# HeadReaper-hc/PL-inertial-slam

Measured on AMD Instinct MI355X. Metric: local-BA iterations/sec (50 KF, 20k pts, 4k lines, IMU), higher is better.
Workload: dtype f64; 1 GPU; configs[2]: 50 KF / 20k points / 4k lines + IMU preintegration edges (9-DoF PVR + 6-DoF bias vertices); K=50, points=20000, lines=4000, point_obs=86023, line_obs=17197, pose_dim=735, dense_dim=357, banded_twisted_solve=False, twin_factorisation=True, fused_landmark_passes=True

## Files before the change

pl-inertial-slam_amd/csrc/plba_api.hip:

```cpp
#include <atomic>
#include <algorithm>
#include <thread>
#include <array>
#include <chrono>
#include <cmath>
#include <cstdio>
#include <cstring>
#include <condition_variable>
#include <functional>
#include <map>
#include <mutex>

#include "plba_problem.h"

using namespace plba;

namespace {
char g_create_err[256] = "";
static std::mutex g_ctx_mu;
static std::vector<HostCtx> g_ctx_free;
static std::map<int, hipStream_t> g_lib_stream;
static std::vector<plba_problem*> g_parked;
static const size_t PARK_MAX = 2;
}
// ... 464 lines not shown
        if (use_lut) for (int w = 0; w < g.nw; ++w) lut[g.kf[w]] = (uint8_t)w;
        int l = g.lm0, ob = H.span_ob0[gi];
        for (int n = H.span_at[gi]; n < H.span_end[gi]; ++n, ++l) {
            const int s = ordall[n];
            o_slot[l] = s; o_fixed[l] = fixed[s]; o_ob0[l] = ob;
            uint8_t* w8 = o_ws8 + (size_t)l * wmax;
            memset(w8, 0xFF, (size_t)wmax);
            int nk = 0;
            for (int e = ls[s]; e < ls[s + 1]; ++e, ++ob, ++nk) {
                int w = 0;
                if (use_lut) w = lut[okf[e]];
                else while (g.kf[w] != okf[e]) ++w;
                bad |= (w8[w] != 0xFF);
                w8[w] = (uint8_t)nk;
                o_orig[ob] = e;
            }
        }
    }
    if (bad) H.bad[t] = 1;
}
static bool lm_groups_finish(LmHost& H) {
    HostPool::get().finish();
    for (int b : H.bad) if (b) return false;
    return true;
}
static void build_lm_groups(const plba_problem* p, const std::vector<int32_t>& lm_start, const std::vector<int32_t>& ob_kf, LmHost& H) {
    const int K = p->win.K, Np = p->win.Np, Nl = p->win.Nl, Ep = p->win.Ep, L = Np + Nl, E = (int)ob_kf.size();
    H.cov.assign((size_t)K * K, 0);
    const bool gt = (p->opt.diag & PLBA_DIAG_TIMING) != 0;
    auto g0 = std::chrono::steady_clock::now();
    auto glap = [&](const char* what) { if (!gt) return; auto t = std::chrono::steady_clock::now(); fprintf(stderr, "[prepare]   groups: %-18s %8.3f ms\n", what, std::chrono::duration<double, std::milli>(t - g0).count()); g0 = t; };
    int nwide_pt = 0, nwide_ln = 0;
    for (int s = 0; s < L; ++s) if (lm_start[s + 1] - lm_start[s] > LMF_W) ++(s < Np ? nwide_pt : nwide_ln);
    const bool any_wide = nwide_pt + nwide_ln > 0;
    int steps = 1;
    {
        static int cus = 0;
        if (!cus) { int dev = 0; if (hipGetDevice(&dev) != hipSuccess || hipDeviceGetAttribute(&cus, hipDeviceAttributeMultiprocessorCount, dev) != hipSuccess || cus < 1) cus = 256; }
        const int slots = 2 * cus;
        const long wg_steps = (Np - nwide_pt + 31) / 32 + (Nl - nwide_ln + 15) / 16 + (nwide_pt + 15) / 16 + (nwide_ln + 7) / 8;
        const long cap1 = std::max<long>(32, (long)(1.12 * cus) - (p->win.M + 1) - (p->win.M / 4 + 1));
        steps = (int)std::max<long>(1, (wg_steps + cap1 - 1) / cap1);
        if (steps > 16) {
            for (int R = 1; R <= 64; ++R) {
                const long cap = (long)(0.97 * R * slots);
                steps = (int)std::max<long>(1, (wg_steps + cap - 1) / cap);
                if (steps <= 16) break;
// ... 106 lines not shown
    H.staged = false;
    if (nob > 20000) {
        H.p_ob_orig = (int32_t*)stage_take(std::max<size_t>(H.n_ob, 1) * 4);
        H.p_lm_slot = (int32_t*)stage_take(std::max<size_t>(H.n_lm, 1) * 4); H.p_lm_ob0 = (int32_t*)stage_take((H.n_lm + 1) * 4);
        H.p_lm_ws8 = (uint8_t*)stage_take(std::max<size_t>(H.n_lm * H.wmax, 1)); H.p_lm_fixed = (uint8_t*)stage_take(std::max<size_t>(H.n_lm, 1));
        H.staged = H.p_ob_orig && H.p_lm_slot && H.p_lm_ob0 && H.p_lm_ws8 && H.p_lm_fixed;
    }
    if (!H.staged) {
        H.lm_slot.resize(nlm); H.lm_ob0.resize(nlm + 1); H.lm_ws8.resize((size_t)nlm * H.wmax); H.lm_fixed.resize(nlm); H.ob_orig.resize(nob);
        H.p_lm_slot = H.lm_slot.data(); H.p_lm_ob0 = H.lm_ob0.data(); H.p_lm_ws8 = H.lm_ws8.data(); H.p_lm_fixed = H.lm_fixed.data(); H.p_ob_orig = H.ob_orig.data();
    }
    H.p_lm_ob0[nlm] = nob;
    const int NT = E > 400000 ? 32 : E > 60000 ? 16 : E > 20000 ? 4 : 1;
    H.gcut.assign(NT + 1, ngrp);
    H.gcut[0] = 0;
    for (int t = 1, g = 0; t < NT; ++t) { while (g < ngrp && H.span_ob0[g] < (int64_t)nob * t / NT) ++g; H.gcut[t] = g; }
    H.bad.assign(NT, 0);
    glap("table allocation");
    const plba_problem* pp = p; const std::vector<int32_t>* ls = &lm_start; const std::vector<int32_t>* ok = &ob_kf; LmHost* Hp = &H;
    HostPool::get().start(NT, [pp, ls, ok, Hp](int t) { lm_fill_groups(pp, *ls, *ok, *Hp, t); });
    {
        size_t npairs_tot = 0, nrows_tot = 0;
        for (const LmGroup& g : H.grp) { int nf = 0; for (int q = 0; q < g.nw; ++q) nf += g.off[q] >= 0; npairs_tot += (size_t)nf * (nf + 1) / 2; nrows_tot += nf; }
        H.blk_c.resize(npairs_tot); H.row_c.resize(nrows_tot);
        auto* bc = H.blk_c.data(); auto* rc = H.row_c.data();
        uint8_t* cov = H.cov.data();
        for (int gi = 0; gi < ngrp; ++gi) {
            const LmGroup& g = H.grp[gi];
            for (int q = 0; q < g.nw; ++q) {
                if (g.off[q] < 0) continue;
                for (int pp = 0; pp <= q; ++pp) {
                    if (g.off[pp] < 0) continue;
                    const int i = g.kf[pp], j = g.kf[q];
                    cov[(size_t)i * K + j] = 1; cov[(size_t)j * K + i] = 1;
                    *bc++ = {(int64_t)i * K + j, gi * H.npair + q * (q + 1) / 2 + pp};
                }
                *rc++ = {(int64_t)g.kf[q], gi * H.wmax + q};
            }
        }
    }
    {
        std::vector<int32_t>& c2 = H.c2; std::vector<int32_t>& pos = H.pos;
        c2.assign((size_t)K * K + 1, 0);
        for (const auto& b : H.blk_c) c2[b.first + 1]++;
        for (size_t k = 0; k < (size_t)K * K; ++k) c2[k + 1] += c2[k];
        H.blk_src.resize(H.blk_c.size());
        for (size_t k = 0; k < (size_t)K * K; ++k) if (c2[k + 1] > c2[k]) { const int i = (int)(k / K), j = (int)(k % K); H.blk_ij.push_back((int32_t)(i | (j << 16))); H.blk_start.push_back(c2[k]); }
        H.blk_start.push_back((int32_t)H.blk_c.size());
        pos.assign(c2.begin(), c2.end() - 1);
        for (const auto& b : H.blk_c) H.blk_src[pos[b.first]++] = b.second;
        c2.assign(K + 1, 0);
        for (const auto& r : H.row_c) c2[r.first + 1]++;
        for (int k = 0; k < K; ++k) c2[k + 1] += c2[k];
        H.row_src.resize(H.row_c.size());
        for (int k = 0; k < K; ++k) if (c2[k + 1] > c2[k]) { H.row_kf.push_back(k); H.row_start.push_back(c2[k]); }
        H.row_start.push_back((int32_t)H.row_c.size());
        pos.assign(c2.begin(), c2.end() - 1);
        for (const auto& r : H.row_c) H.row_src[pos[r.first]++] = r.second;
    }
    glap("gather lists");
// ... 1901 lines not shown
        const int o = w == "err_pvr" ? 0 : 9, nn = w == "err_pvr" ? 9 : 6;
        v.resize((size_t)p->win.M * nn);
        for (int m = 0; m < p->win.M; ++m) memcpy(&v[(size_t)m * nn], &h[(size_t)m * 16 + o], nn * 8);
    } else if (w == "err_prior") { HIPCK(p, fetch(d.pr_err, p->pr_nv ? p->pr_n : 0, v)); }
    else if ((w == "err_pt" || w == "err_ln") && p->lm_ok) {
        std::vector<double> h; HIPCK(p, fetch(p->d_ob_err.p, 2 * (size_t)p->E, h));
        if (w == "err_pt") v.assign(h.begin(), h.begin() + 2 * (size_t)p->win.Ep);
        else { v.assign((size_t)p->win.El * 3, 0.0); for (int e = 0; e < p->win.El; ++e) { v[3 * (size_t)e] = h[2 * (size_t)(p->win.Ep + e)]; v[3 * (size_t)e + 1] = h[2 * (size_t)(p->win.Ep + e) + 1]; } }
    }
    else if (w == "err_pt" || w == "err_ln") {
        std::vector<double> h; HIPCK(p, fetch(d.erec, ((size_t)p->win.Ep + 2 * (size_t)p->win.El) * EREC_UNIT, h));
        if (w == "err_pt") { v.resize((size_t)p->win.Ep * 2); for (int e = 0; e < p->win.Ep; ++e) { const size_t o = (size_t)p->ob_pos[e] * EREC_UNIT; v[2 * (size_t)e] = h[o + EREC_PT_E0]; v[2 * (size_t)e + 1] = h[o + EREC_PT_E0 + 1]; } }
        else { v.assign((size_t)p->win.El * 3, 0.0); for (int e = 0; e < p->win.El; ++e) { const size_t o = (size_t)p->ob_pos[p->win.Ep + e] * EREC_UNIT; v[3 * (size_t)e] = h[o + 13]; v[3 * (size_t)e + 1] = h[o + 14]; } }
    } else if (w == "erec") {
        if (p->lm_ok) FAIL(p, PLBA_ERR_STATE, "\"erec\": the fused landmark passes keep no record table");
        HIPCK(p, fetch(d.erec, ((size_t)p->win.Ep + 2 * (size_t)p->win.El) * EREC_UNIT, v));
    }
    else if (w == "stamps") { HIPCK(p, fetch(d.maxd_part, 80, v)); }
    else if (w == "dbgbuf") { HIPCK(p, fetch(d.dbgbuf, 128, v)); }
    else if (w == "pose_dim") v = {(double)p->P};
    else if (w == "marg_path") v.assign(p->marg_path, p->marg_path + 5);
    else if (w == "prof_lin_launches") v = {(double)p->prof_lin_launches};
    else if (w == "lm_groups") v = p->lm_hist;
    else if (w == "lm_fused") v = {(double)(p->lm_ok ? 1 : 0), (double)p->lv.ngrp, (double)p->lv.nblk, p->lm_ok && p->lm_hist.size() > 18 ? p->lm_hist[18] : 0.0 };
    else if (w == "marg_J") v = p->marg_dbg;
    else if (w == "dense_dim") v = {(double)(p->chain_ok ? p->cv.Pd : p->P)};
    else if (w == "band") v = {(double)(p->band_ok ? 1 : 0)};
    else if (w == "twin") v = {(double)(p->twin_ok ? 1 : 0)};
    else if (w == "solver_plan") {
        const bool ninv = !p->band_ok && (p->chain_ok ? p->dd.Ninv : p->dv.Ninv) != nullptr;
        v = {(double)(p->band_ok ? 3 : p->twin_ok ? 2 : p->chain_ok ? 1 : 0), (double)((p->chain_ok ? p->cv.Pdpad : p->Ppad) / 32), ninv ? 1.0 : 0.0, (double)p->plan_hbt,
             p->plan_twin[0], p->plan_twin[1], p->plan_twin[2], p->plan_twin[3], p->plan_twin[4], (double)(p->band_ok ? p->bandv.nA : 0), (double)(p->band_ok ? p->bandv.nB : 0)};
    }
    else if (w == "fact_launches_estimate") v = {(double)p->seg_launch_est};
    else if (w == "fact_launches") {
        if (p->band_ok) v = {2.0};
        else if (p->twin_ok) v = {(double)(p->twinv.nlaunch + (p->twinv.T - p->twinv.m0 - 1))};
        else v = {-1.0};
    }
    else if (w == "chi2") { HIPCK(p, plba_d2h(p, p->h_ctrl, d.ctrl, sizeof(Ctrl))); v = {p->h_ctrl->current_chi}; }
    else if (w == "maxdiag") { HIPCK(p, plba_d2h(p, p->h_ctrl, d.ctrl, sizeof(Ctrl))); v = {p->h_ctrl->maxdiag}; }
    else if (w == "solver_ok") { HIPCK(p, plba_d2h(p, p->h_ctrl, d.ctrl, sizeof(Ctrl))); v = {(double)p->h_ctrl->solver_ok}; }
    else FAIL(p, PLBA_ERR_INVALID, "debug_get: unknown buffer '%s'", what);
    if (n) *n = v.size();
    if (out) { const size_t c = std::min(v.size(), cap); if (c) memcpy(out, v.data(), c * 8); }
    return PLBA_OK;
// ... 4 lines not shown
```

pl-inertial-slam_amd/csrc/plba_internal.h:

```cpp
#pragma once
#include <hip/hip_runtime.h>
#include <stdint.h>
#include <map>
#include <mutex>
#include <string>
#include <utility>
#include <vector>

#include "plba.h"
#include "plba_math.h"

namespace plba {

constexpr int TILE = 64;

inline hipError_t ensure_dyn_lds(const void* func, int bytes) {
    static std::mutex mu;
    static std::map<std::pair<int, const void*>, int> done;
    int dev = 0;
    hipError_t e = hipGetDevice(&dev);
    if (e != hipSuccess) return e;
    std::lock_guard<std::mutex> lk(mu);
    auto it = done.find({dev, func});
    if (it != done.end() && it->second >= bytes) return hipSuccess;
// ... 69 lines not shown
    int band;
    int twin_m0;
    const int32_t* cs_order;
    const int32_t* twin_fac;
    const int32_t* perm;
    const int32_t* xmap;
    double* wtw;
    double* alt2;
    double* alt;
    int flow;
    int wide;
    double *chi_part, *scale_part, *maxd_part, *kfdiag, *posediag;
    Ctrl* ctrl;
    plba_trace_row* trace;
    int trace_cap;
    int* trace_n;
};

struct Robust { int on[5]; double delta[5]; };

constexpr int LMF_W = 8;
constexpr int LMF_W2 = 16;
struct LmGroup { int32_t lm0, nlm, nw, kind ; int32_t kf[LMF_W2]; int32_t off[LMF_W2]; };
struct LmView {
    int ngrp;
    const LmGroup* grp;
    const int32_t* lm_slot;
    const int32_t* lm_ob0;
    const int32_t* ob_orig;
    double* ob_chi_g;
    int wmax, npair, part_stride;
    const uint8_t* lm_ws8;
    const uint8_t* lm_fixed_g;
    uint8_t* ob_level_g;
    const double* meas_pt;
    const double* meas_ln;
    const double* ob_wt;
    double* part;
    int nblk;
    const int32_t* blk_ij;
    const int32_t* blk_start;
    const int32_t* blk_src;
    int nrow;
    const int32_t* row_kf;
    const int32_t* row_start;
    const int32_t* row_src;
// ... 106 lines not shown
```

pl-inertial-slam_amd/csrc/plba_kernels.hip:

```cpp
#include "plba_internal.h"
#include "plba_chain_dev.h"

namespace plba {

#define DEV __device__ __forceinline__

DEV double wave_sum(double v) {
#pragma unroll
    for (int o = 32; o > 0; o >>= 1) v += __shfl_down(v, o, 64);
    return v;
}
DEV double wave_max(double v) {
#pragma unroll
    for (int o = 32; o > 0; o >>= 1) v = fmax(v, __shfl_down(v, o, 64));
    return v;
}
DEV double block_sum_256(double v, double* s4) {
    v = wave_sum(v);
    int w = threadIdx.x >> 6;
    if ((threadIdx.x & 63) == 0) s4[w] = v;
    __syncthreads();
    double r = 0;
    if (threadIdx.x == 0) r = (s4[0] + s4[1]) + (s4[2] + s4[3]);
    __syncthreads();
// ... 1497 lines not shown
    hipLaunchKernelGGL(k_reduce, dim3(1), dim3(256), 0, s, d, nred, nred, owns_pose_edges ? 1 : 0, red);
}
void launch_posediag(const DevBuf& d, hipStream_t s) {
    hipLaunchKernelGGL(k_posediag, dim3((d.ld + 255) / 256), dim3(256), 0, s, d);
    hipLaunchKernelGGL(k_posediag_kf, dim3((d.K * 6 + 255) / 256), dim3(256), 0, s, d);
}
__global__ __launch_bounds__(256) void k_lm_lambda_init(DevBuf d, LmView lv, LmParams lp, double* red, int iteration, int nred) {
    __shared__ double s4[4];
    __shared__ double s_part[256];
    reduce_inline(d, nred, nred, red, s4);
    for (int r = threadIdx.x; r < d.ld; r += 256) d.posediag[r] = (r < d.P) ? d.Himu[(size_t)r * d.ld + r] + d.Hconst[(size_t)r * d.ld + r] : 0.0;
    __syncthreads();
    const int nent = lv.nrow * 6;
    const int nch = nent > 0 && nent <= 128 ? 256 / nent : 1;
    for (int base = 0; base < nent; base += 256) {
        const int idx = base + (int)threadIdx.x % (nch > 1 ? nent : 256), ch = nch > 1 ? (int)threadIdx.x / nent : 0;
        double v = 0.0;
        const bool live = idx < nent && ch < nch;
        int k = 0, c = 0;
        if (live) {
            k = idx / 6; c = idx - 6 * k;
            for (int q = lv.row_start[k] + ch; q < lv.row_start[k + 1]; q += nch) {
                const int src = lv.row_src[q];
                v += lv.part[(size_t)(src / lv.wmax) * lv.part_stride + lv.npair * 36 + (src % lv.wmax) * 12 + c];
            }
        }
        if (nch > 1) {
            s_part[threadIdx.x] = v;
            __syncthreads();
            if (live && ch == 0) { v = 0.0; for (int q = 0; q < nch; ++q) v += s_part[q * nent + idx]; }
        }
        if (live && ch == 0) {
            const int kf = lv.row_kf[k], o = d.kf_off_pvr[kf];
            d.kfdiag[kf * 6 + c] = v;
            if (o >= 0) d.posediag[o + pmap(c)] += v;
        }
    }
    __syncthreads();
    double md = 0.0;
    for (int r = threadIdx.x; r < d.P; r += 256) md = fmax(md, fabs(d.posediag[r]));
    double mx = block_max_256(md, s4);
    if (threadIdx.x == 0) {
        Ctrl* c = d.ctrl;
        c->current_chi = red[0];
        c->iteration = iteration;
        c->trial = 0;
        mx = fmax(mx, red[2]);
// ... 148 lines not shown
```

pl-inertial-slam_amd/csrc/plba_lm_dev.h:

```cpp
#pragma once

namespace plba {

typedef double double4v_lm __attribute__((ext_vector_type(4)));

constexpr int LMF_UNITS = 32;
constexpr int LMF_ROWS = 6 * LMF_W;
constexpr int LMF_SCOLS = 3 * LMF_UNITS;
constexpr int LMF_HCOLS = 2 * LMF_UNITS;
struct LmLds {
    double kc[2][LMF_W2][KFCAM_STRIDE];
    double xs[LMF_W2][6];
    double red[4][8];
    int koff[LMF_W2];
};
struct LmAcc {
    double op[4 * 24 * LMF_ROWS];
};

DEV double quad_or_sum(double v) { return quad_sum(v); }
DEV int quad_or_i(int v) {
    v |= __builtin_amdgcn_update_dpp(0, v, 0xB1, 0xf, 0xf, false);
    v |= __builtin_amdgcn_update_dpp(0, v, 0x4E, 0xf, 0xf, false);
    v |= __builtin_amdgcn_update_dpp(0, v, 0x141, 0xf, 0xf, false);
    return v;
}
DEV double shfl_xor8(double v) {
    return dpp_get<0x128, 0xf>(v);
}

DEV double lm_rcp(double x) {
    double y = __builtin_amdgcn_rcp(x);
    double e = fma(-x, y, 1.0);
    y = fma(y, e, y);
    e = fma(-x, y, 1.0);
    return fma(y, e, y);
}
DEV double lm_rsqrt(double x) {
    double y = __builtin_amdgcn_rsq(x);
    const double hx = 0.5 * x;
    y = y * fma(-hx * y, y, 1.5);
// ... 113 lines not shown
    if (s.has) {
        s.orig = lv.ob_err ? lv.ob_orig[s.e] : 0; s.wt = lv.ob_wt[s.e];
        s.lvl0 = lv.ob_level_g[s.e] == 0;
        if (IS_LINE) { const double* m = lv.meas_ln + (size_t)(s.e - d.Ep) * 3; s.meas[0] = m[0]; s.meas[1] = m[1]; s.meas[2] = m[2]; }
        else { const double2 m = reinterpret_cast<const double2*>(lv.meas_pt)[s.e]; s.meas[0] = m.x; s.meas[1] = m.y; }
    }
}
template <bool IS_LINE, bool WIDE = false>
DEV void lm_load(const DevBuf& d, const LmView& lv, const LmHead& g, int state, int step, int wv, int lane, LmStep& s) {
    LmIdx x;
    lm_load_idx<IS_LINE, WIDE>(lv, g, step, wv, lane, x);
    lm_load_data<IS_LINE, WIDE>(d, lv, state, lane, x, s);
}

DEV void lm_stage_window(const DevBuf& d, const LmGroup* gp, int nw, int state, LmLds& S) {
    if ((int)threadIdx.x < LMF_W2) {
        const int p = threadIdx.x;
        if (p < nw) { kfcam_make(d.cam, d.kf[state] + (size_t)gp->kf[p] * KF_STRIDE, S.kc[0][p]); S.koff[p] = gp->off[p]; }
        else { for (int t = 0; t < KFCAM_STRIDE; ++t) S.kc[0][p][t] = 0.0; S.koff[p] = -1; }
    }
}

constexpr int LMF_WCOLS = 24;
constexpr int LMF_NVEC = 33;
DEV void lm_wave_sync() {
    __builtin_amdgcn_fence(__ATOMIC_RELEASE, "wavefront");
    __builtin_amdgcn_wave_barrier();
    __builtin_amdgcn_fence(__ATOMIC_ACQUIRE, "wavefront");
}
template <bool IS_LINE, int MODE>
DEV void lm_schur_group(const DevBuf& d, const LmView& lv, const int gidx, const int state, const Robust& rb, LmLds& S, LmAcc& A4) {
    constexpr int NR = IS_LINE ? 1 : 2;
    const LmGroup* gp = lv.grp + gidx;
    const LmHead g = lm_head(*gp);
    const int wv = threadIdx.x >> 6, lane = threadIdx.x & 63, sub = lane & 7, li = lane & 15, lk = lane >> 4, u8 = lane >> 3;
    const double lambda = MODE == 0 ? d.ctrl->lambda : 0.0;
    lm_stage_window(d, gp, g.nw, state, S);
    const int nunits = IS_LINE ? 2 * g.nlm : g.nlm;
    const int nsteps = (nunits + LMF_UNITS - 1) / LMF_UNITS;
#ifdef PLBA_STAMPS_LMF
    unsigned long long fs[12] = {0,0,0,0,0,0,0,0,0,0,0,0}; fs[0] = __builtin_readcyclecounter();
#define FSTAMP(i) do { if (step == 0) fs[i] = __builtin_readcyclecounter(); } while (0)
#define FSTAMP1(i) fs[i] = __builtin_readcyclecounter()
#else
#define FSTAMP(i) do {} while (0)
#define FSTAMP1(i) do {} while (0)
#endif
    LmStep cur;
    lm_load<IS_LINE>(d, lv, g, state, 0, wv, lane, cur);
    LmIdx ix1;
    ix1.uvalid = false; ix1.slot = 0; ix1.e = 0; ix1.has = false; ix1.fixed = true;
    if (nsteps > 1) lm_load_idx<IS_LINE>(lv, g, 1, wv, lane, ix1);
    __syncthreads();
    const double* kc = S.kc[0][sub];
    const bool kfree = S.koff[sub] >= 0;
    const double4v_lm z4 = (double4v_lm){0.0, 0.0, 0.0, 0.0};
    double4v_lm a00 = z4, a10 = z4, a11 = z4, a20 = z4, a21 = z4, a22 = z4;
    double vec[LMF_NVEC];
#pragma unroll
    for (int t = 0; t < LMF_NVEC; ++t) vec[t] = 0.0;
    double chi_acc = 0.0, maxd = 0.0;
    double* op = A4.op + wv * (LMF_WCOLS * LMF_ROWS);
    for (int step = 0; step < nsteps; ++step) {
        FSTAMP(1);
        LmRows<NR> r;
        const int rowsel = IS_LINE ? (u8 & 1) : 0;
        lm_eval<IS_LINE, NR>(d, rb, kc, cur.has && kfree, cur.L, cur.meas, cur.wt, cur.has, cur.lvl0, rowsel, true, r);
        FSTAMP(2);
        double h[6], b[3];
        int nact;
        lm_hll<NR>(r, h, b, nact);
        FSTAMP(3);
        const bool active = cur.uvalid && nact > 0 && !cur.fixed;
        if (!IS_LINE || rowsel == 0) chi_acc += r.rho;
        if (MODE == 1 && r.act && (!IS_LINE || rowsel == 0)) {
            lv.ob_chi_g[cur.e] = r.chi;
            if (lv.ob_err) { lv.ob_err[2 * (size_t)cur.orig] = r.e[0]; }
        }
        if (MODE == 1 && lv.ob_err && r.act) lv.ob_err[2 * (size_t)cur.orig + (IS_LINE ? rowsel : 1)] = r.e[NR - 1];
        if (lv.dbg_out && cur.uvalid && sub == 0) {
            const int dslot = lv.lm_grouped ? lv.lm_slot[cur.slot] : cur.slot;
            double* ho = d.hll + (size_t)dslot * 12 + (IS_LINE ? 6 * rowsel : 0);
            double* bo = d.bl + (size_t)dslot * 6 + (IS_LINE ? 3 * rowsel : 0);
#pragma unroll
            for (int t = 0; t < 6; ++t) ho[t] = h[t];
// ... 44 lines not shown
                }
                double q = 0.0;
#pragma unroll
                for (int a = 0; a < NR; ++a) q += r.j[a][c] * es[a];
                vec[21 + c] -= q;
                vec[27 + c] += A3[0] * y[0] + A3[1] * y[1] + A3[2] * y[2];
#pragma unroll
                for (int c2 = 0; c2 <= c; ++c2) {
                    double hq = 0.0;
#pragma unroll
                    for (int a = 0; a < NR; ++a) hq += r.j[a][c] * r.j[a][c2];
#ifndef PLBA_X_NOH
                    vec[hidx++] += hq;
#else
                    (void)hq; (void)hidx;
#endif
                }
            }
            FSTAMP(4);
            LmStep nxt;
            if (step + 1 < nsteps) lm_load_data<IS_LINE>(d, lv, state, lane, ix1, nxt);
            if (step + 2 < nsteps) lm_load_idx<IS_LINE>(lv, g, step + 2, wv, lane, ix1);
            lm_wave_sync();
#pragma unroll 2
            for (int s4 = 0; s4 < LMF_WCOLS / 4; ++s4) {
                const double* col = op + (4 * s4 + lk) * LMF_ROWS + li;
                const double f0 = col[0], f1 = col[16], f2 = col[32];
#ifdef PLBA_X_NOMFMA
                a00[0] += f0 * f1 * f2;
                continue;
#endif
                a00 = __builtin_amdgcn_mfma_f64_16x16x4f64(f0, f0, a00, 0, 0, 0);
                a10 = __builtin_amdgcn_mfma_f64_16x16x4f64(f1, f0, a10, 0, 0, 0);
                a11 = __builtin_amdgcn_mfma_f64_16x16x4f64(f1, f1, a11, 0, 0, 0);
                a20 = __builtin_amdgcn_mfma_f64_16x16x4f64(f2, f0, a20, 0, 0, 0);
                a21 = __builtin_amdgcn_mfma_f64_16x16x4f64(f2, f1, a21, 0, 0, 0);
                a22 = __builtin_amdgcn_mfma_f64_16x16x4f64(f2, f2, a22, 0, 0, 0);
            }
            FSTAMP(5);
            lm_wave_sync();
            cur = nxt;
        }
        FSTAMP(7);
    }
    FSTAMP1(8);
#pragma unroll
    for (int t = 0; t < LMF_NVEC; ++t) {
        double v = vec[t];
        v += shfl_xor8(v);
        v += __shfl_xor(v, 16);
        v += __shfl_xor(v, 32);
        vec[t] = v;
    }
    chi_acc = wave_sum(chi_acc); maxd = wave_max(maxd);
    __syncthreads();
    double* cb = A4.op;
    double* vs = A4.op + 2 * 6 * 256;
    if (lane < LMF_W) {
#pragma unroll
        for (int t = 0; t < LMF_NVEC; ++t) vs[(wv * LMF_W + lane) * LMF_NVEC + t] = vec[t];
    }
    if (lane == 0) { S.red[wv][0] = chi_acc; S.red[wv][1] = maxd; }
    if (MODE == 0) {
        double* mine = cb + (wv & 1) * (6 * 256);
        if (wv < 2) {
#pragma unroll
            for (int v4 = 0; v4 < 4; ++v4) {
                const int o = (lk + 4 * v4) * 16 + li;
                mine[0 * 256 + o] = a00[v4]; mine[1 * 256 + o] = a10[v4]; mine[2 * 256 + o] = a11[v4];
                mine[3 * 256 + o] = a20[v4]; mine[4 * 256 + o] = a21[v4]; mine[5 * 256 + o] = a22[v4];
            }
        }
        __syncthreads();
        if (wv >= 2) {
#pragma unroll
            for (int v4 = 0; v4 < 4; ++v4) {
                const int o = (lk + 4 * v4) * 16 + li;
                mine[0 * 256 + o] += a00[v4]; mine[1 * 256 + o] += a10[v4]; mine[2 * 256 + o] += a11[v4];
                mine[3 * 256 + o] += a20[v4]; mine[4 * 256 + o] += a21[v4]; mine[5 * 256 + o] += a22[v4];
            }
        }
    }
    __syncthreads();
    FSTAMP1(9);
    double* part = lv.part + (size_t)gidx * lv.part_stride;
    if (MODE == 0) {
        for (int idx = threadIdx.x; idx < 36 * 36; idx += 256) {
            const int t = idx / 36, rc = idx - t * 36, r = rc / 6, c = rc - r * 6;
            const int q = (t >= 28) ? 7 : (t >= 21) ? 6 : (t >= 15) ? 5 : (t >= 10) ? 4 : (t >= 6) ? 3 : (t >= 3) ? 2 : (t >= 1) ? 1 : 0;
            const int p = t - q * (q + 1) / 2;
            int a = 6 * p + r, b2 = 6 * q + c;
            if (a < b2) { const int tmp = a; a = b2; b2 = tmp; }
            const int ta = a >> 4, tb = b2 >> 4;
            const int o = (ta * (ta + 1) / 2 + tb) * 256 + (a & 15) * 16 + (b2 & 15);
            const double sv = cb[o] + cb[6 * 256 + o];
            double hv = 0.0;
            if (p == q) {
                const int hr = r >= c ? r : c, hc = r >= c ? c : r, k = hr * (hr + 1) / 2 + hc;
                hv = (vs[(0 * LMF_W + p) * LMF_NVEC + k] + vs[(1 * LMF_W + p) * LMF_NVEC + k]) + (vs[(2 * LMF_W + p) * LMF_NVEC + k] + vs[(3 * LMF_W + p) * LMF_NVEC + k]);
            }
            part[idx] = hv - sv;
        }
    }
    if ((int)threadIdx.x < LMF_W * 12 && (MODE == 0 || threadIdx.x % 12 < 6)) {
        const int p = threadIdx.x / 12, k = 21 + threadIdx.x % 12;
        part[lv.npair * 36 + threadIdx.x] = (vs[(0 * LMF_W + p) * LMF_NVEC + k] + vs[(1 * LMF_W + p) * LMF_NVEC + k]) + (vs[(2 * LMF_W + p) * LMF_NVEC + k] + vs[(3 * LMF_W + p) * LMF_NVEC + k]);
    }
    if (threadIdx.x == 0) {
        d.chi_part[gidx] = (S.red[0][0] + S.red[1][0]) + (S.red[2][0] + S.red[3][0]);
        if (MODE == 1) d.maxd_part[gidx] = fmax(fmax(S.red[0][1], S.red[1][1]), fmax(S.red[2][1], S.red[3][1]));
    }
#ifdef PLBA_STAMPS_LMF
    asm volatile("s_waitcnt vmcnt(0)" ::: "memory");
    FSTAMP1(10);
    if (MODE == 0 && threadIdx.x == 0 && (gidx == 0 || gidx == lv.ngrp / 2 || gidx == lv.ngrp - 1)) {
        const int o = gidx == 0 ? 0 : gidx == lv.ngrp / 2 ? 16 : 32;
        for (int q = 0; q < 11; ++q) d.dbgbuf[o + q] = (double)(fs[q] - fs[0]);
        d.dbgbuf[o + 11] = (double)nsteps; d.dbgbuf[o + 12] = (double)(long long)__builtin_amdgcn_s_memrealtime();
    }
#endif
}

__device__ const signed char LMW_TILE[2][4][6][2] = {
// ... 172 lines not shown
        }
    }
    if ((int)threadIdx.x < LMF_W2 * 12 && (MODE == 0 || threadIdx.x % 12 < 6)) {
        const int pslot = threadIdx.x / 12, k = 21 + threadIdx.x % 12;
        part[lv.npair * 36 + threadIdx.x] = (vs[(0 * LMF_W2 + pslot) * LMF_NVEC + k] + vs[(1 * LMF_W2 + pslot) * LMF_NVEC + k]) + (vs[(2 * LMF_W2 + pslot) * LMF_NVEC + k] + vs[(3 * LMF_W2 + pslot) * LMF_NVEC + k]);
    }
    if (threadIdx.x == 0) {
        d.chi_part[gidx] = (S.red[0][0] + S.red[1][0]) + (S.red[2][0] + S.red[3][0]);
        if (MODE == 1) d.maxd_part[gidx] = fmax(fmax(S.red[0][1], S.red[1][1]), fmax(S.red[2][1], S.red[3][1]));
    }
}

DEV void lm_gather_part(const DevBuf& d, const LmView& lv, int add_lambda, int bid, int tid, double* s_red ) {
    const double lambda = d.ctrl->lambda;
    const int ld = d.ld;
    if (bid < lv.nblk) {
        const int b = bid, rc = tid % 36, ch = tid / 36;
        const int n0 = lv.blk_start[b], n1 = lv.blk_start[b + 1];
        double a0 = 0.0, a1 = 0.0;
        if (ch < 7) {
            int s = n0 + ch;
            for (; s + 7 < n1; s += 14) {
                const int src0 = lv.blk_src[s], src1 = lv.blk_src[s + 7];
                a0 += lv.part[(size_t)(src0 / lv.npair) * lv.part_stride + (src0 % lv.npair) * 36 + rc];
                a1 += lv.part[(size_t)(src1 / lv.npair) * lv.part_stride + (src1 % lv.npair) * 36 + rc];
            }
            if (s < n1) { const int src0 = lv.blk_src[s]; a0 += lv.part[(size_t)(src0 / lv.npair) * lv.part_stride + (src0 % lv.npair) * 36 + rc]; }
        }
        s_red[tid] = a0 + a1;
        __syncthreads();
        if (tid >= 36) return;
        const int ij = lv.blk_ij[b], i = ij & 0xffff, j = (ij >> 16) & 0xffff;
        const int r = rc / 6, c = rc % 6;
        const size_t e0 = (size_t)(d.kf_off_pvr[i] + pmap(r)) * ld + d.kf_off_pvr[j] + pmap(c);
        const size_t e1 = (size_t)(d.kf_off_pvr[j] + pmap(c)) * ld + d.kf_off_pvr[i] + pmap(r);
        double v = d.Himu[e0] + d.Hconst[e0];
        if (i == j && r == c && add_lambda) v += lambda;
        double sum = 0.0;
#pragma unroll
        for (int q = 0; q < 7; ++q) sum += s_red[q * 36 + rc];
        v += sum;
        d.sys[e0] = v; d.Himu_alt[e0] = 0.0;
        if (i != j) { d.sys[e1] = v; d.Himu_alt[e1] = 0.0; }
        return;
    }
    const int k = bid - lv.nblk;
    if (k >= lv.nrow) return;
    const int t = tid % 12, ch = tid / 12;
    const int n0 = lv.row_start[k], n1 = lv.row_start[k + 1];
    double acc = 0.0;
    if (ch < 21)
        for (int s = n0 + ch; s < n1; s += 21) {
            const int src = lv.row_src[s];
            acc += lv.part[(size_t)(src / lv.wmax) * lv.part_stride + lv.npair * 36 + (src % lv.wmax) * 12 + t];
        }
    s_red[tid] = acc;
    __syncthreads();
    if (tid >= 6) return;
    double bp = 0.0, bs = 0.0;
#pragma unroll
    for (int q = 0; q < 21; ++q) { bp += s_red[q * 12 + tid]; bs += s_red[q * 12 + 6 + tid]; }
    const int col = d.kf_off_pvr[lv.row_kf[k]] + pmap(tid);
    const double base = d.bimu[col] + d.bprior[col];
    d.sys[(size_t)d.Ppad * ld + col] = base + bp - bs;
    d.sys[(size_t)(d.Ppad + 1) * ld + col] = base + bp; d.bpg[col] = base + bp; d.bimu_alt[col] = 0.0;
}
__host__ __device__ inline int lm_gather_blocks(const LmView& lv) { return lv.nblk + lv.nrow; }
DEV void lm_gather_diag(const DevBuf& d, const LmView& lv, int bid, int tid, double* s_red) {
    const int k = bid;
    if (k >= lv.nrow) return;
    const int t = tid % 12, ch = tid / 12;
    double acc = 0.0;
    if (ch < 21 && t < 6)
        for (int s = lv.row_start[k] + ch; s < lv.row_start[k + 1]; s += 21) {
            const int src = lv.row_src[s];
            acc += lv.part[(size_t)(src / lv.wmax) * lv.part_stride + lv.npair * 36 + (src % lv.wmax) * 12 + t];
        }
    s_red[tid] = acc;
    __syncthreads();
    if (tid >= 6) return;
    double v = 0.0;
#pragma unroll
    for (int q = 0; q < 21; ++q) v += s_red[q * 12 + tid];
    d.kfdiag[lv.row_kf[k] * 6 + tid] = v;
}
DEV void lm_assemble_rest(const DevBuf& d, const LmView& lv, int add_lambda, int bid, int nblocks, int tid, int nthreads) {
    const double lambda = d.ctrl->lambda;
    const int n = lv.nalist2;
    const size_t stride = (size_t)nblocks * nthreads;
    for (size_t k = (size_t)bid * nthreads + tid; k < (size_t)n + (size_t)d.ld; k += stride) {
        if (k < (size_t)n) {
            const int idx = lv.alist2[k];
            const int r = idx / d.ld, c = idx - r * d.ld;
            double v = d.Himu[idx] + d.Hconst[idx];
            if (r == c && add_lambda) v += (r < d.P) ? lambda : 1.0;
            d.Himu_alt[idx] = 0.0;
            d.sys[idx] = v;
        } else {
            const int c = (int)(k - n);
// ... 115 lines not shown
```

pl-inertial-slam_amd/csrc/plba_problem.h:

```cpp
#pragma once
#include <algorithm>
#include <chrono>
#include <cstring>
#include <map>
#include <mutex>
#include <utility>
#include <vector>

#include "plba_internal.h"
#include "plba_window.h"

namespace plba {

struct DevPool {
    static constexpr size_t POOL_CAP = (size_t)8 << 30;
    std::mutex mu;
    std::map<std::pair<int, size_t>, std::vector<void*>> free_;
    size_t cached = 0;
    size_t n_malloc = 0, n_reuse = 0;
    static size_t size_class(size_t bytes) { size_t c = 4096; while (c < bytes) c <<= 1; return c; }
    hipError_t get(size_t bytes, void** out, size_t* cls) {
        int dev = 0;
        (void)hipGetDevice(&dev);
        *cls = size_class(bytes);
// ... 134 lines not shown
    hipError_t upload_staged(const T* src, size_t cnt) {
        hipError_t e = alloc(cnt, cnt == 0);
        if (e != hipSuccess || cnt == 0) return e;
        return hipMemcpyAsync(p, src, cnt * sizeof(T), hipMemcpyHostToDevice, darr_stream());
    }
    void release() { if (p && !batched) dev_pool().put(p, cls); p = nullptr; n = 0; cls = 0; batched = false; }
    void swap(DArr& o) { std::swap(p, o.p); std::swap(n, o.n); std::swap(cls, o.cls); std::swap(batched, o.batched); std::swap(bgen, o.bgen); std::swap(bsrc, o.bsrc); }
    DArr() = default;
    DArr(const DArr&) = delete;
    DArr& operator=(const DArr&) = delete;
    ~DArr() { release(); }
};

}

namespace plba {
struct MargPending;
struct LmHost {
    std::vector<LmGroup> grp;
    int wmax = 8, npair = 36;
    std::vector<int32_t> lm_slot, lm_ob0, ob_orig, blk_ij, blk_start, blk_src, row_kf, row_start, row_src;
    std::vector<uint8_t> lm_ws8, lm_fixed, cov;
    bool staged = false;
    int32_t *p_lm_slot = nullptr, *p_lm_ob0 = nullptr, *p_ob_orig = nullptr;
    uint8_t *p_lm_ws8 = nullptr, *p_lm_fixed = nullptr;
    size_t n_lm = 0, n_ob = 0, n_meas_pt = 0, n_meas_ln = 0;
    std::vector<int32_t> kmin, kmax, ord, tmp, cnt, ordall, stamp, span_at, span_end, span_ob0, gcut, bad, c2, pos;
    std::vector<std::pair<int64_t, int32_t>> blk_c, row_c;
    std::vector<uint64_t> kmask;
};
}

struct HostCtx {
    int device = 0;
    hipStream_t stream = nullptr;
    void* h_ctrl = nullptr;
    void* h_mail = nullptr;
    void* d_mail = nullptr;
    plba::StageArea* stage = nullptr;
    plba::LmHost* lm_host = nullptr;
    plba::StageArea* slide_stage = nullptr;
    plba::StageArea* marg_stage = nullptr;
};


struct plba_problem {
// ... 184 lines not shown
```

Before: 7777 iterations/s.

## Skip empty MFMA tiles, precompute gather offsets, and per-wave landmark partial reduction

The fused landmark kernel ballots which keyframe slots are occupied and skips the MFMA tile products for empty 16-row tiles. Each wave now writes its accumulators and vector sums into its own LDS region, which removes a block-wide barrier and the two-phase add. A constexpr table replaces the per-element index arithmetic in the output write. The gather index tables now store absolute element offsets into the partial buffer instead of group/pair indices, so the gather kernels avoid integer division and modulo. Host code falls back when those offsets would overflow int32, and several debug query endpoints are added.

```diff
diff --git a/pl-inertial-slam_amd/csrc/plba_api.hip b/pl-inertial-slam_amd/csrc/plba_api.hip
--- a/pl-inertial-slam_amd/csrc/plba_api.hip
+++ b/pl-inertial-slam_amd/csrc/plba_api.hip
@@ -510,7 +510,7 @@
 static bool lm_groups_finish(LmHost& H) {
     HostPool::get().finish();
     for (int b : H.bad) if (b) return false;
-    return true;
+    return !H.too_big;
 }
 static void build_lm_groups(const plba_problem* p, const std::vector<int32_t>& lm_start, const std::vector<int32_t>& ob_kf, LmHost& H) {
     const int K = p->win.K, Np = p->win.Np, Nl = p->win.Nl, Ep = p->win.Ep, L = Np + Nl, E = (int)ob_kf.size();
@@ -663,10 +663,13 @@
     {
         size_t npairs_tot = 0, nrows_tot = 0;
         for (const LmGroup& g : H.grp) { int nf = 0; for (int q = 0; q < g.nw; ++q) nf += g.off[q] >= 0; npairs_tot += (size_t)nf * (nf + 1) / 2; nrows_tot += nf; }
+        const int pstride = H.npair * 36 + H.wmax * 12;
+        H.too_big = (int64_t)ngrp * pstride > INT32_MAX;
+        if (H.too_big) npairs_tot = nrows_tot = 0;
         H.blk_c.resize(npairs_tot); H.row_c.resize(nrows_tot);
         auto* bc = H.blk_c.data(); auto* rc = H.row_c.data();
         uint8_t* cov = H.cov.data();
-        for (int gi = 0; gi < ngrp; ++gi) {
+        for (int gi = 0; gi < ngrp && !H.too_big; ++gi) {
             const LmGroup& g = H.grp[gi];
             for (int q = 0; q < g.nw; ++q) {
                 if (g.off[q] < 0) continue;
@@ -674,9 +677,9 @@
                     if (g.off[pp] < 0) continue;
                     const int i = g.kf[pp], j = g.kf[q];
                     cov[(size_t)i * K + j] = 1; cov[(size_t)j * K + i] = 1;
-                    *bc++ = {(int64_t)i * K + j, gi * H.npair + q * (q + 1) / 2 + pp};
+                    *bc++ = {(int64_t)i * K + j, gi * pstride + (q * (q + 1) / 2 + pp) * 36};
                 }
-                *rc++ = {(int64_t)g.kf[q], gi * H.wmax + q};
+                *rc++ = {(int64_t)g.kf[q], gi * pstride + H.npair * 36 + q * 12};
             }
         }
     }
@@ -2624,6 +2627,51 @@
     else if (w == "marg_path") v.assign(p->marg_path, p->marg_path + 5);
     else if (w == "prof_lin_launches") v = {(double)p->prof_lin_launches};
     else if (w == "lm_groups") v = p->lm_hist;
+    else if (w == "lm_out_map") { static constexpr LmOutMap om = lm_out_map_make(); v.assign(om.e, om.e + 36 * 36); }
+    else if (w == "lm_gather_src") {
+        if (!p->lm_ok) FAIL(p, PLBA_ERR_STATE, "\"lm_gather_src\": the window does not run the fused landmark passes");
+        const LmView& lv = p->lv;
+        v = {(double)lv.npair, (double)lv.wmax, (double)lv.part_stride, (double)lv.nblk, (double)lv.nrow};
+        std::vector<int32_t> key, st, src;
+        for (int pass = 0; pass < 2; ++pass) {
+            const int n = pass ? lv.nrow : lv.nblk;
+            key.resize((size_t)n); st.resize((size_t)n + 1);
+            if (n) HIPCK(p, plba_d2h(p, key.data(), pass ? lv.row_kf : lv.blk_ij, key.size() * 4));
+            HIPCK(p, plba_d2h(p, st.data(), pass ? lv.row_start : lv.blk_start, st.size() * 4));
+            src.resize((size_t)st[n]);
+            if (!src.empty()) HIPCK(p, plba_d2h(p, src.data(), pass ? lv.row_src : lv.blk_src, src.size() * 4));
+            v.insert(v.end(), key.begin(), key.end()); v.insert(v.end(), st.begin(), st.end()); v.insert(v.end(), src.begin(), src.end());
+        }
+    }
+    else if (w == "lm_group_win") {
+        if (!p->lm_ok) FAIL(p, PLBA_ERR_STATE, "\"lm_group_win\": the window does not run the fused landmark passes");
+        std::vector<LmGroup> grp((size_t)p->lv.ngrp);
+        HIPCK(p, plba_d2h(p, grp.data(), p->lv.grp, grp.size() * sizeof(LmGroup)));
+        for (const LmGroup& g : grp) { v.push_back(g.kind); v.push_back(g.nw); for (int q = 0; q < LMF_W2; ++q) v.push_back(g.kf[q]); for (int q = 0; q < LMF_W2; ++q) v.push_back(g.off[q]); }
+    }
+    else if (w == "lm_tile_skip") {
+        if (!p->lm_ok) FAIL(p, PLBA_ERR_STATE, "\"lm_tile_skip\": the window does not run the fused landmark passes");
+        const LmView& lv = p->lv;
+        std::vector<LmGroup> grp((size_t)lv.ngrp);
+        HIPCK(p, plba_d2h(p, grp.data(), lv.grp, grp.size() * sizeof(LmGroup)));
+        size_t nlm = 0;
+        for (const LmGroup& g : grp) nlm = std::max(nlm, (size_t)g.lm0 + g.nlm);
+        std::vector<uint8_t> ws((size_t)nlm * lv.wmax);
+        if (!ws.empty()) HIPCK(p, plba_d2h(p, ws.data(), lv.lm_ws8, ws.size()));
+        v.assign(11, 0.0);
+        for (const LmGroup& g : grp) {
+            if (g.kind & 2) continue;
+            const int per = (g.kind & 1) ? 2 : 1, nunits = per * g.nlm, nsteps = (nunits + 31) / 32;
+            for (int wsx = 0; wsx < 4 * nsteps; ++wsx) {
+                int occ = 0;
+                for (int u = 8 * wsx; u < 8 * wsx + 8 && u < nunits; ++u)
+                    for (int q = 0; q < LMF_W; ++q)
+                        if (ws[(size_t)(g.lm0 + u / per) * lv.wmax + q] != 0xFF) occ |= (q <= 2 ? 1 : 0) | (q >= 2 && q <= 5 ? 2 : 0) | (q >= 5 ? 4 : 0);
+                const int nt = (occ & 1) + ((occ >> 1) & 1) + ((occ >> 2) & 1);
+                v[0] += 1.0; v[1] += nt * (nt + 1) / 2; v[2] += 6.0; v[3 + occ] += 1.0;
+            }
+        }
+    }
     else if (w == "lm_fused") v = {(double)(p->lm_ok ? 1 : 0), (double)p->lv.ngrp, (double)p->lv.nblk, p->lm_ok && p->lm_hist.size() > 18 ? p->lm_hist[18] : 0.0 };
     else if (w == "marg_J") v = p->marg_dbg;
     else if (w == "dense_dim") v = {(double)(p->chain_ok ? p->cv.Pd : p->P)};
diff --git a/pl-inertial-slam_amd/csrc/plba_internal.h b/pl-inertial-slam_amd/csrc/plba_internal.h
--- a/pl-inertial-slam_amd/csrc/plba_internal.h
+++ b/pl-inertial-slam_amd/csrc/plba_internal.h
@@ -115,6 +115,24 @@
 constexpr int LMF_W = 8;
 constexpr int LMF_W2 = 16;
 struct LmGroup { int32_t lm0, nlm, nw, kind ; int32_t kf[LMF_W2]; int32_t off[LMF_W2]; };
+constexpr int LMF_NVEC = 33;
+struct LmOutMap { uint32_t e[36 * 36]; };
+constexpr LmOutMap lm_out_map_make() {
+    LmOutMap m{};
+    for (int q = 0, t = 0; q < LMF_W; ++q)
+        for (int p = 0; p <= q; ++p, ++t)
+            for (int r = 0; r < 6; ++r)
+                for (int c = 0; c < 6; ++c) {
+                    int a = 6 * p + r, b = 6 * q + c;
+                    if (a < b) { const int tmp = a; a = b; b = tmp; }
+                    const int ta = a >> 4, tb = b >> 4;
+                    const uint32_t o = (uint32_t)((ta * (ta + 1) / 2 + tb) * 256 + (a & 15) * 16 + (b & 15));
+                    const int hr = r >= c ? r : c, hc = r >= c ? c : r;
+                    const uint32_t dg = p == q ? (uint32_t)(1 + p * LMF_NVEC + hr * (hr + 1) / 2 + hc) : 0u;
+                    m.e[t * 36 + r * 6 + c] = o | (dg << 11);
+                }
+    return m;
+}
 struct LmView {
     int ngrp;
     const LmGroup* grp;
diff --git a/pl-inertial-slam_amd/csrc/plba_kernels.hip b/pl-inertial-slam_amd/csrc/plba_kernels.hip
--- a/pl-inertial-slam_amd/csrc/plba_kernels.hip
+++ b/pl-inertial-slam_amd/csrc/plba_kernels.hip
@@ -1543,7 +1543,7 @@
             k = idx / 6; c = idx - 6 * k;
             for (int q = lv.row_start[k] + ch; q < lv.row_start[k + 1]; q += nch) {
                 const int src = lv.row_src[q];
-                v += lv.part[(size_t)(src / lv.wmax) * lv.part_stride + lv.npair * 36 + (src % lv.wmax) * 12 + c];
+                v += lv.part[src + c];
             }
         }
         if (nch > 1) {
diff --git a/pl-inertial-slam_amd/csrc/plba_lm_dev.h b/pl-inertial-slam_amd/csrc/plba_lm_dev.h
--- a/pl-inertial-slam_amd/csrc/plba_lm_dev.h
+++ b/pl-inertial-slam_amd/csrc/plba_lm_dev.h
@@ -14,9 +14,12 @@
     double red[4][8];
     int koff[LMF_W2];
 };
+constexpr int LMF_WREG = 6 * 256;
 struct LmAcc {
-    double op[4 * 24 * LMF_ROWS];
+    double op[4 * LMF_WREG];
+    double vs[4 * LMF_W * LMF_NVEC];
 };
+__device__ const LmOutMap LM_OUT_MAP = lm_out_map_make();
 
 DEV double quad_or_sum(double v) { return quad_sum(v); }
 DEV int quad_or_i(int v) {
@@ -176,7 +179,6 @@
 }
 
 constexpr int LMF_WCOLS = 24;
-constexpr int LMF_NVEC = 33;
 DEV void lm_wave_sync() {
     __builtin_amdgcn_fence(__ATOMIC_RELEASE, "wavefront");
     __builtin_amdgcn_wave_barrier();
@@ -214,7 +216,8 @@
 #pragma unroll
     for (int t = 0; t < LMF_NVEC; ++t) vec[t] = 0.0;
     double chi_acc = 0.0, maxd = 0.0;
-    double* op = A4.op + wv * (LMF_WCOLS * LMF_ROWS);
+    static_assert(LMF_WCOLS * LMF_ROWS <= LMF_WREG, "a wave's operand panel lies inside its own region");
+    double* op = A4.op + wv * LMF_WREG;
     for (int step = 0; step < nsteps; ++step) {
         FSTAMP(1);
         LmRows<NR> r;
@@ -305,20 +308,24 @@
             if (step + 1 < nsteps) lm_load_data<IS_LINE>(d, lv, state, lane, ix1, nxt);
             if (step + 2 < nsteps) lm_load_idx<IS_LINE>(lv, g, step + 2, wv, lane, ix1);
             lm_wave_sync();
+            const unsigned long long hb = __builtin_amdgcn_ballot_w64(cur.has);
+            const bool o1 = (hb & 0x3C3C3C3C3C3C3C3Cull) != 0, o2 = (hb & 0xE0E0E0E0E0E0E0E0ull) != 0;
 #pragma unroll 2
             for (int s4 = 0; s4 < LMF_WCOLS / 4; ++s4) {
                 const double* col = op + (4 * s4 + lk) * LMF_ROWS + li;
-                const double f0 = col[0], f1 = col[16], f2 = col[32];
-#ifdef PLBA_X_NOMFMA
-                a00[0] += f0 * f1 * f2;
-                continue;
-#endif
+                const double f0 = col[0];
                 a00 = __builtin_amdgcn_mfma_f64_16x16x4f64(f0, f0, a00, 0, 0, 0);
-                a10 = __builtin_amdgcn_mfma_f64_16x16x4f64(f1, f0, a10, 0, 0, 0);
-                a11 = __builtin_amdgcn_mfma_f64_16x16x4f64(f1, f1, a11, 0, 0, 0);
-                a20 = __builtin_amdgcn_mfma_f64_16x16x4f64(f2, f0, a20, 0, 0, 0);
-                a21 = __builtin_amdgcn_mfma_f64_16x16x4f64(f2, f1, a21, 0, 0, 0);
-                a22 = __builtin_amdgcn_mfma_f64_16x16x4f64(f2, f2, a22, 0, 0, 0);
+                if (o1) {
+                    const double f1 = col[16];
+                    a10 = __builtin_amdgcn_mfma_f64_16x16x4f64(f1, f0, a10, 0, 0, 0);
+                    a11 = __builtin_amdgcn_mfma_f64_16x16x4f64(f1, f1, a11, 0, 0, 0);
+                }
+                if (o2) {
+                    const double f2 = col[32];
+                    a20 = __builtin_amdgcn_mfma_f64_16x16x4f64(f2, f0, a20, 0, 0, 0);
+                    if (o1) a21 = __builtin_amdgcn_mfma_f64_16x16x4f64(f2, col[16], a21, 0, 0, 0);
+                    a22 = __builtin_amdgcn_mfma_f64_16x16x4f64(f2, f2, a22, 0, 0, 0);
+                }
             }
             FSTAMP(5);
             lm_wave_sync();
@@ -327,61 +334,52 @@
         FSTAMP(7);
     }
     FSTAMP1(8);
-#pragma unroll
-    for (int t = 0; t < LMF_NVEC; ++t) {
-        double v = vec[t];
-        v += shfl_xor8(v);
-        v += __shfl_xor(v, 16);
-        v += __shfl_xor(v, 32);
-        vec[t] = v;
+    double* own = A4.op + wv * LMF_WREG;
+#pragma unroll
+    for (int t = 0; t < LMF_NVEC; ++t) vec[t] += shfl_xor8(vec[t]);
+    if ((lane & 8) == 0) {
+#pragma unroll
+        for (int t = 0; t < LMF_NVEC; ++t) own[((lane >> 4) * LMF_W + sub) * LMF_NVEC + t] = vec[t];
+    }
+    unsigned omap[6] = {0, 0, 0, 0, 0, 0};
+    if (MODE == 0) {
+#pragma unroll
+        for (int k = 0; k < 6; ++k) if (k < 5 || threadIdx.x < 36 * 36 - 5 * 256) omap[k] = LM_OUT_MAP.e[threadIdx.x + 256 * k];
     }
     chi_acc = wave_sum(chi_acc); maxd = wave_max(maxd);
-    __syncthreads();
-    double* cb = A4.op;
-    double* vs = A4.op + 2 * 6 * 256;
-    if (lane < LMF_W) {
-#pragma unroll
-        for (int t = 0; t < LMF_NVEC; ++t) vs[(wv * LMF_W + lane) * LMF_NVEC + t] = vec[t];
+    lm_wave_sync();
+    constexpr int NV8 = LMF_W * LMF_NVEC;
+    static_assert(4 * NV8 <= LMF_WREG, "the rows' sums fit the wave's region");
+#pragma unroll
+    for (int k = 0; k < (NV8 + 63) / 64; ++k) {
+        const int j = lane + 64 * k;
+        if (j < NV8) A4.vs[wv * NV8 + j] = (own[j] + own[NV8 + j]) + (own[2 * NV8 + j] + own[3 * NV8 + j]);
     }
     if (lane == 0) { S.red[wv][0] = chi_acc; S.red[wv][1] = maxd; }
+    FSTAMP1(6);
     if (MODE == 0) {
-        double* mine = cb + (wv & 1) * (6 * 256);
-        if (wv < 2) {
-#pragma unroll
-            for (int v4 = 0; v4 < 4; ++v4) {
-                const int o = (lk + 4 * v4) * 16 + li;
-                mine[0 * 256 + o] = a00[v4]; mine[1 * 256 + o] = a10[v4]; mine[2 * 256 + o] = a11[v4];
-                mine[3 * 256 + o] = a20[v4]; mine[4 * 256 + o] = a21[v4]; mine[5 * 256 + o] = a22[v4];
-            }
-        }
-        __syncthreads();
-        if (wv >= 2) {
-#pragma unroll
-            for (int v4 = 0; v4 < 4; ++v4) {
-                const int o = (lk + 4 * v4) * 16 + li;
-                mine[0 * 256 + o] += a00[v4]; mine[1 * 256 + o] += a10[v4]; mine[2 * 256 + o] += a11[v4];
-                mine[3 * 256 + o] += a20[v4]; mine[4 * 256 + o] += a21[v4]; mine[5 * 256 + o] += a22[v4];
-            }
+        lm_wave_sync();
+#pragma unroll
+        for (int v4 = 0; v4 < 4; ++v4) {
+            const int o = (lk + 4 * v4) * 16 + li;
+            own[0 * 256 + o] = a00[v4]; own[1 * 256 + o] = a10[v4]; own[2 * 256 + o] = a11[v4];
+            own[3 * 256 + o] = a20[v4]; own[4 * 256 + o] = a21[v4]; own[5 * 256 + o] = a22[v4];
         }
     }
     __syncthreads();
     FSTAMP1(9);
+    const double* cb = A4.op;
+    const double* vs = A4.vs;
     double* part = lv.part + (size_t)gidx * lv.part_stride;
     if (MODE == 0) {
-        for (int idx = threadIdx.x; idx < 36 * 36; idx += 256) {
-            const int t = idx / 36, rc = idx - t * 36, r = rc / 6, c = rc - r * 6;
-            const int q = (t >= 28) ? 7 : (t >= 21) ? 6 : (t >= 15) ? 5 : (t >= 10) ? 4 : (t >= 6) ? 3 : (t >= 3) ? 2 : (t >= 1) ? 1 : 0;
-            const int p = t - q * (q + 1) / 2;
-            int a = 6 * p + r, b2 = 6 * q + c;
-            if (a < b2) { const int tmp = a; a = b2; b2 = tmp; }
-            const int ta = a >> 4, tb = b2 >> 4;
-            const int o = (ta * (ta + 1) / 2 + tb) * 256 + (a & 15) * 16 + (b2 & 15);
-            const double sv = cb[o] + cb[6 * 256 + o];
+#pragma unroll
+        for (int k = 0; k < 6; ++k) {
+            const int idx = threadIdx.x + 256 * k;
+            if (k == 5 && idx >= 36 * 36) break;
+            const int o = omap[k] & 0x7ff, dg = (int)(omap[k] >> 11);
+            const double sv = (cb[o] + cb[2 * LMF_WREG + o]) + (cb[LMF_WREG + o] + cb[3 * LMF_WREG + o]);
             double hv = 0.0;
-            if (p == q) {
-                const int hr = r >= c ? r : c, hc = r >= c ? c : r, k = hr * (hr + 1) / 2 + hc;
-                hv = (vs[(0 * LMF_W + p) * LMF_NVEC + k] + vs[(1 * LMF_W + p) * LMF_NVEC + k]) + (vs[(2 * LMF_W + p) * LMF_NVEC + k] + vs[(3 * LMF_W + p) * LMF_NVEC + k]);
-            }
+            if (dg) hv = (vs[dg - 1] + vs[NV8 + dg - 1]) + (vs[2 * NV8 + dg - 1] + vs[3 * NV8 + dg - 1]);
             part[idx] = hv - sv;
         }
     }
@@ -600,10 +598,10 @@
             int s = n0 + ch;
             for (; s + 7 < n1; s += 14) {
                 const int src0 = lv.blk_src[s], src1 = lv.blk_src[s + 7];
-                a0 += lv.part[(size_t)(src0 / lv.npair) * lv.part_stride + (src0 % lv.npair) * 36 + rc];
-                a1 += lv.part[(size_t)(src1 / lv.npair) * lv.part_stride + (src1 % lv.npair) * 36 + rc];
-            }
-            if (s < n1) { const int src0 = lv.blk_src[s]; a0 += lv.part[(size_t)(src0 / lv.npair) * lv.part_stride + (src0 % lv.npair) * 36 + rc]; }
+                a0 += lv.part[src0 + rc];
+                a1 += lv.part[src1 + rc];
+            }
+            if (s < n1) { const int src0 = lv.blk_src[s]; a0 += lv.part[src0 + rc]; }
         }
         s_red[tid] = a0 + a1;
         __syncthreads();
@@ -630,7 +628,7 @@
     if (ch < 21)
         for (int s = n0 + ch; s < n1; s += 21) {
             const int src = lv.row_src[s];
-            acc += lv.part[(size_t)(src / lv.wmax) * lv.part_stride + lv.npair * 36 + (src % lv.wmax) * 12 + t];
+            acc += lv.part[src + t];
         }
     s_red[tid] = acc;
     __syncthreads();
@@ -652,7 +650,7 @@
     if (ch < 21 && t < 6)
         for (int s = lv.row_start[k] + ch; s < lv.row_start[k + 1]; s += 21) {
             const int src = lv.row_src[s];
-            acc += lv.part[(size_t)(src / lv.wmax) * lv.part_stride + lv.npair * 36 + (src % lv.wmax) * 12 + t];
+            acc += lv.part[src + t];
         }
     s_red[tid] = acc;
     __syncthreads();
diff --git a/pl-inertial-slam_amd/csrc/plba_problem.h b/pl-inertial-slam_amd/csrc/plba_problem.h
--- a/pl-inertial-slam_amd/csrc/plba_problem.h
+++ b/pl-inertial-slam_amd/csrc/plba_problem.h
@@ -180,6 +180,7 @@
     std::vector<int32_t> lm_slot, lm_ob0, ob_orig, blk_ij, blk_start, blk_src, row_kf, row_start, row_src;
     std::vector<uint8_t> lm_ws8, lm_fixed, cov;
     bool staged = false;
+    bool too_big = false;
     int32_t *p_lm_slot = nullptr, *p_lm_ob0 = nullptr, *p_ob_orig = nullptr;
     uint8_t *p_lm_ws8 = nullptr, *p_lm_fixed = nullptr;
     size_t n_lm = 0, n_ob = 0, n_meas_pt = 0, n_meas_ln = 0;
```

Result: slower. 7593 iterations/s (-2.4%).
